# CyberAgentAILab/layout-dm

Hardware: NVIDIA H100
Metric: layouts_per_sec_T100_batch1024_N25 (higher is better)
Workload: dtype fp16

## Files before the change

### layoutdm_b200/csrc/common.cuh

```cuda
#pragma once
#include <cuda.h>
#include <cuda_bf16.h>
#include <cuda_fp16.h>
#include <cuda_runtime.h>
#include <stdint.h>

namespace ldm {

#define LDM_DEVINL __device__ __forceinline__

constexpr float kLogEps = -69.07755278982137f;

LDM_DEVINL uint32_t smem_u32(const void* p) { return static_cast<uint32_t>(__cvta_generic_to_shared(p)); }
LDM_DEVINL void st_shared_u32(uint32_t addr, uint32_t v) { asm volatile("st.shared.u32 [%0], %1;" ::"r"(addr), "r"(v) : "memory"); }

LDM_DEVINL void pdl_wait() { asm volatile("griddepcontrol.wait;" ::: "memory"); }
LDM_DEVINL void pdl_launch_dependents() { asm volatile("griddepcontrol.launch_dependents;" ::: "memory"); }
LDM_DEVINL void pdl_sync() { pdl_wait(); pdl_launch_dependents(); }

LDM_DEVINL void mbar_init(uint64_t* bar, uint32_t count) {
  asm volatile("mbarrier.init.shared::cta.b64 [%0], %1;" ::"r"(smem_u32(bar)), "r"(count) : "memory");
}
LDM_DEVINL void fence_mbar_init() { asm volatile("fence.mbarrier_init.release.cluster;" ::: "memory"); }

// ... 35 lines not shown
               ::"l"(reinterpret_cast<uint64_t>(map)), "r"(smem_u32(smem_src)), "r"(c0), "r"(c1)
               : "memory");
}
LDM_DEVINL void bulk_copy_g2s(void* smem_dst, const void* src, uint32_t bytes, uint64_t* bar) {
  asm volatile("cp.async.bulk.shared::cluster.global.mbarrier::complete_tx::bytes [%0], [%1], %2, [%3];"
               ::"r"(smem_u32(smem_dst)), "l"(reinterpret_cast<uint64_t>(src)), "r"(bytes), "r"(smem_u32(bar))
               : "memory");
}
LDM_DEVINL void bulk_copy_s2g(void* dst, const void* smem_src, uint32_t bytes) {
  asm volatile("cp.async.bulk.global.shared::cta.bulk_group [%0], [%1], %2;"
               ::"l"(reinterpret_cast<uint64_t>(dst)), "r"(smem_u32(smem_src)), "r"(bytes)
               : "memory");
}
LDM_DEVINL void bulk_commit_group() { asm volatile("cp.async.bulk.commit_group;" ::: "memory"); }
template <int N>
LDM_DEVINL void bulk_wait_group_read() { asm volatile("cp.async.bulk.wait_group.read %0;" ::"n"(N) : "memory"); }
LDM_DEVINL void bulk_wait_group_all() { asm volatile("cp.async.bulk.wait_group 0;" ::: "memory"); }
LDM_DEVINL void fence_proxy_async_smem() { asm volatile("fence.proxy.async.shared::cta;" ::: "memory"); }

template <int R>
LDM_DEVINL void setmaxnreg_inc() { asm volatile("setmaxnreg.inc.sync.aligned.u32 %0;" ::"n"(R)); }
template <int R>
LDM_DEVINL void setmaxnreg_dec() { asm volatile("setmaxnreg.dec.sync.aligned.u32 %0;" ::"n"(R)); }

LDM_DEVINL void named_bar_sync(int id, int nthreads) { asm volatile("bar.sync %0, %1;" ::"r"(id), "r"(nthreads) : "memory"); }
LDM_DEVINL void named_bar_arrive(int id, int nthreads) { asm volatile("bar.arrive %0, %1;" ::"r"(id), "r"(nthreads) : "memory"); }

LDM_DEVINL void wgmma_fence() { asm volatile("wgmma.fence.sync.aligned;" ::: "memory"); }
LDM_DEVINL void wgmma_commit() { asm volatile("wgmma.commit_group.sync.aligned;" ::: "memory"); }
template <int N>
LDM_DEVINL void wgmma_wait() { asm volatile("wgmma.wait_group.sync.aligned %0;" ::"n"(N) : "memory"); }
template <int N>
LDM_DEVINL void fence_acc(float (&d)[N]) {
#pragma unroll
  for (int i = 0; i < N; ++i) asm volatile("" : "+f"(d[i])::"memory");
}

template <int SW>
LDM_DEVINL uint64_t make_smem_desc(uint32_t smem_addr) {
  static_assert(SW == 128 || SW == 64, "the kernels use the 128- and 64-byte swizzles");
  uint64_t d = 0;
  d |= static_cast<uint64_t>((smem_addr & 0x3FFFF) >> 4);
  d |= static_cast<uint64_t>(1) << 16;
  d |= static_cast<uint64_t>(8 * SW >> 4) << 32;
  d |= static_cast<uint64_t>(SW == 128 ? 1 : 2) << 62;
  return d;
// ... 215 lines not shown
```

### layoutdm_b200/csrc/gemm_tc.cuh

```cuda
#pragma once
#include "common.cuh"

namespace ldm {

constexpr int kBM = 128;
constexpr int kWgK = 16;
constexpr int kGemmConsumers = 256;
constexpr int kProducerRegs = 40, kConsumerRegs = 232;

constexpr int gemm_kb(bool split) { return split ? 32 : 64; }

enum : int { EPI_QKV = 0, EPI_RELU = 1, EPI_F32 = 2, EPI_LN = 3 };

struct GemmParams {
  int M, N, K;
  int n_tiles;
  const float* bias;
  void* out;
  int ldo;
  float qscale;
  int qcols;
  const float* resid;
  float* y_out;
  const float* ln_scale;
// ... 437 lines not shown
          for (int h = 0; h < 2; ++h) {
            float v[4];
            bias_act<EPI>(acc[h], j8, p.bias, c, scale, v);
            st_shared_u32(blk + (h * 64 + rw) * 128, O::pack(v[0], v[1]));
            st_shared_u32(blk + (h * 64 + rw + 8) * 128, O::pack(v[2], v[3]));
          }
        }
        fence_proxy_async_smem();
        wg_bar();
        if (leader) {
          tma_store_2d(&map_out, stage, n0 + cb * 64, m0);
          bulk_commit_group();
        }
      }
    }
    if (!mine_any) {
      for (int kb = 0; kb < num_kb; ++kb) { mbar_wait(&a_full[kb], ip); mbar_arrive(&a_empty[kb]); }
    }
  }
  if (leader) bulk_wait_group_all();
}

constexpr int kLnThreads = 384, kLnEpiThreads = 96;
struct LnSmem {
  static constexpr int kRows = 64, kWgCols = 232, kCols = 2 * kWgCols;
  using R = Ring<32, 1, kRows, kWgCols, 2, 3, false>;
  static constexpr int kLd = kCols + 8;
  static constexpr int kOffBuf = R::kBytes;
  static constexpr int kOffBars = kOffBuf + kRows * kLd * 4;
  static constexpr int kOffStat = kOffBars + 64;
  static constexpr int kBytes = kOffStat + 3 * kRows * 4 + 1024 ;
  static_assert(kLd * 4 % 16 == 0, "bulk copies need 16-byte aligned rows");
  static_assert(kBytes <= 232448, "exceeds the 227 KB of shared memory per CTA");
};

template <int MODE>
__global__ void __launch_bounds__(kLnThreads, 1)
gemm_ln_kernel(const __grid_constant__ OpMaps<MODE> map_a , const __grid_constant__ OpMaps<MODE> map_b ,
               const GemmParams p) {
  static_assert(!kOpSplit<MODE>, "the split mode runs the fragment-epilogue LN GEMM");
  using SM = LnSmem;
  using O = OpT<MODE>;
  constexpr int kRows = SM::kRows, kWgCols = SM::kWgCols, kLd = SM::kLd, kAcc = kWgCols / 2;
  constexpr int kEpi = kGemmConsumers, kProducer = kEpi + kLnEpiThreads;

  extern __shared__ __align__(1024) uint8_t smem_raw[];
  uint8_t* smem = reinterpret_cast<uint8_t*>((reinterpret_cast<uintptr_t>(smem_raw) + 1023) & ~uintptr_t(1023));
  SM::R ring(smem, reinterpret_cast<uint64_t*>(smem + SM::kOffBars));
  uint64_t* res_full = ring.empty + SM::R::kStages;
  uint64_t* buf_full = res_full + 1;
  float* buf = reinterpret_cast<float*>(smem + SM::kOffBuf);
  float* s_piv = reinterpret_cast<float*>(smem + SM::kOffStat);
  float* s_sum = s_piv + kRows;
  float* s_rstd = s_sum + kRows;

  const int warp = __shfl_sync(0xffffffffu, threadIdx.x >> 5, 0), lane = threadIdx.x & 31;
  const int N = p.N;
  const int num_kb = SM::R::num_kb(p.K);
  const int n_work = p.M / kRows;
  const auto tile_m0 = [&](int t) { return (p.rev ? n_work - 1 - t : t) * kRows; };

  if (threadIdx.x == kProducer) {
    ring.prefetch(map_a, map_b);
    ring.init();
    mbar_init(res_full, 1);
    mbar_init(buf_full, kGemmConsumers);
    fence_mbar_init();
  }
  __syncthreads();
  pdl_sync();

  if (threadIdx.x >= kProducer) {
    if (threadIdx.x == kProducer) {
      uint32_t phase = 0;
      int s = 0;
      for (int t = blockIdx.x; t < n_work; t += gridDim.x) ring.load_tile(s, phase, map_a, map_b, num_kb, tile_m0(t), 0);
    }
    return;
  }

  if (threadIdx.x >= kEpi) {
    const int et = threadIdx.x - kEpi;
    const bool copier = et < 32;
    const uint32_t row_bytes = static_cast<uint32_t>(N) * sizeof(float);
    const float inv_n = 1.0f / static_cast<float>(N);
    constexpr int kVec = kWgCols / 2;
    constexpr int kTotal = kRows * kVec;
    constexpr int kPerThread = (kTotal + kLnEpiThreads - 1) / kLnEpiThreads;
    const auto load_resid = [&](int t) {
      if (lane == 0) mbar_arrive_expect_tx(res_full, kRows * row_bytes);
      __syncwarp();
      const float* src = p.resid + static_cast<size_t>(tile_m0(t)) * N;
      for (int r = lane; r < kRows; r += 32) bulk_copy_g2s(buf + r * kLd, src + static_cast<size_t>(r) * N, row_bytes, res_full);
    };
    const auto store_rows = [&](float* dst) {
      for (int r = lane; r < kRows; r += 32) bulk_copy_s2g(dst + static_cast<size_t>(r) * N, buf + r * kLd, row_bytes);
      bulk_commit_group();
    };
    if (copier) load_resid(blockIdx.x);
    uint32_t bphase = 0;
    for (int t = blockIdx.x; t < n_work; t += gridDim.x) {
      const int m0 = tile_m0(t);
      mbar_wait(buf_full, bphase);
      if (copier && p.y_out != nullptr) store_rows(p.y_out + static_cast<size_t>(m0) * N);
      {
        const int h = (lane >> 2) & 1, q = lane & 3;
#pragma unroll 1
        for (int g = et >> 5; g < kRows / 4; g += kLnEpiThreads / 32) {
          const int r = 4 * g + (lane >> 3);
          const float piv = s_piv[r];
          const float* yr = buf + r * kLd + h * kWgCols + 2 * q;
          float s = 0.0f;
#pragma unroll
          for (int j = 0; j < kWgCols / 8; ++j) {
            const float2 y = *reinterpret_cast<const float2*>(yr + 8 * j);
            s += (y.x - piv) + (y.y - piv);
          }
          s += __shfl_xor_sync(0xffffffffu, s, 1);
          s += __shfl_xor_sync(0xffffffffu, s, 2);
          s += __shfl_xor_sync(0xffffffffu, s, 4);
          float v = 0.0f;
#pragma unroll
          for (int j = 0; j < kWgCols / 8; ++j) {
            const float2 y = *reinterpret_cast<const float2*>(yr + 8 * j);
            const float d0 = fmaf(-s, inv_n, y.x - piv), d1 = fmaf(-s, inv_n, y.y - piv);
            v = fmaf(d0, d0, fmaf(d1, d1, v));
          }
          v += __shfl_xor_sync(0xffffffffu, v, 1);
          v += __shfl_xor_sync(0xffffffffu, v, 2);
          v += __shfl_xor_sync(0xffffffffu, v, 4);
          if ((lane & 7) == 0) { s_sum[r] = s; s_rstd[r] = 1.0f / sqrtf(fmaxf(v * inv_n, 0.0f) + 1e-5f); }
        }
      }
      if (copier) bulk_wait_group_read<0>();
      named_bar_sync(1, kLnEpiThreads);
      const LnAffine a = ln_affine(p.ln_scale, p.ln_shift, p.adaln, p.t_layout, p.n_layouts, m0, N);
      typename O::T* out16 = static_cast<typename O::T*>(p.out);
      const bool keep32 = p.out32 != nullptr;
#pragma unroll 6
      for (int k = 0; k < kPerThread; ++k) {
        const int i = k * kLnEpiThreads + et, r = i / kVec, c = (i - r * kVec) * 4;
        if (i >= kTotal) continue;
        float4* bp = reinterpret_cast<float4*>(buf + r * kLd + c);
        const float4 y = *bp;
        const float4 g = __ldg(reinterpret_cast<const float4*>(a.gam + c)), b = __ldg(reinterpret_cast<const float4*>(a.bet + c));
        const float piv = s_piv[r], s = s_sum[r], rstd = s_rstd[r];
        const float4 v = make_float4(fmaf(fmaf(-s, inv_n, y.x - piv) * rstd, g.x + a.gadd, b.x), fmaf(fmaf(-s, inv_n, y.y - piv) * rstd, g.y + a.gadd, b.y),
                                     fmaf(fmaf(-s, inv_n, y.z - piv) * rstd, g.z + a.gadd, b.z), fmaf(fmaf(-s, inv_n, y.w - piv) * rstd, g.w + a.gadd, b.w));
        *reinterpret_cast<uint2*>(out16 + static_cast<size_t>(m0 + r) * N + c) = make_uint2(O::pack(v.x, v.y), O::pack(v.z, v.w));
        if (keep32) *bp = v;
      }
      if (keep32) fence_proxy_async_smem();
      named_bar_sync(1, kLnEpiThreads);
      if (copier) {
        if (keep32) store_rows(p.out32 + static_cast<size_t>(m0) * N);
        bulk_wait_group_read<0>();
        if (t + static_cast<int>(gridDim.x) < n_work) load_resid(t + gridDim.x);
      }
      bphase ^= 1;
    }
    if (copier) bulk_wait_group_all();
    return;
  }

  const int wn = warp >> 2;
  float acc[kAcc];
  int s = 0;
  uint32_t phase = 0, bphase = 0;
  const int rw = (warp & 3) * 16 + (lane >> 2);
  const int cw = wn * kWgCols + 2 * (lane & 3);
  float* bw = buf + rw * kLd + cw;
  for (int t = blockIdx.x; t < n_work; t += gridDim.x) {
    ring.mma_tile<MODE>(s, phase, acc, 0, wn, num_kb, p.K);
    mbar_wait(res_full, bphase);
    if (cw == 0) { const float b0 = __ldg(p.bias); s_piv[rw] = b0 + bw[0]; s_piv[rw + 8] = b0 + bw[8 * kLd]; }
#pragma unroll
    for (int j = 0; j < kAcc / 4; ++j) {
      const float2 b = __ldg(reinterpret_cast<const float2*>(p.bias + cw + 8 * j));
      float2* y0 = reinterpret_cast<float2*>(bw + 8 * j);
      float2* y1 = reinterpret_cast<float2*>(bw + 8 * kLd + 8 * j);
      const float2 r0 = *y0, r1 = *y1;
      *y0 = make_float2(acc[4 * j] + (b.x + r0.x), acc[4 * j + 1] + (b.y + r0.y));
      *y1 = make_float2(acc[4 * j + 2] + (b.x + r1.x), acc[4 * j + 3] + (b.y + r1.y));
    }
    fence_proxy_async_smem();
    mbar_arrive(buf_full);
    bphase ^= 1;
  }
}

}
```

### layoutdm_b200/csrc/ldm_b200.cu

```cuda
#include <cuda.h>
#include <cuda_runtime.h>

#include <algorithm>
#include <cmath>
#include <cstdarg>
#include <cstdio>
#include <cstdlib>
#include <cstring>
#include <type_traits>
#include <vector>

#include "../../include/ldm_b200.h"
#include "attention.cuh"
#include "common.cuh"
#include "embed.cuh"
#include "gemm_tc.cuh"
#include "posterior_sample.cuh"
#include "relation.cuh"

using namespace ldm;

namespace {

thread_local char g_err[512] = "";
int fail(int code, const char* fmt, ...) {
  va_list ap; va_start(ap, fmt); vsnprintf(g_err, sizeof(g_err), fmt, ap); va_end(ap);
  return code;
}
#define CK(call)                                                                                   \
  do {                                                                                             \
    cudaError_t e__ = (call);                                                                      \
    if (e__ != cudaSuccess) return fail(LDM_ERR_CUDA, "%s failed: %s (%s:%d)", #call, cudaGetErrorString(e__), __FILE__, __LINE__); \
  } while (0)

constexpr int kMaxLayers = 16;
constexpr int kHeadPad = 64;
constexpr int kQkvN = 3 * 8 * kHeadPad;
constexpr int kAttN = 8 * kHeadPad;
constexpr int kMaxLayouts = 32767;
constexpr int kLogitLd = 160;
constexpr int kDModel = 464;
constexpr int kPlainBN = 256, kPlainStages = 4;
constexpr int kRbCols = RbSmem::kCols;
static_assert(kDModel <= RbSmem::kAKb * RbSmem::kKB && kAttN % kRbCols == 0 && kQkvN % 64 == 0 && 4 * kDModel % 64 == 0,
              "row-block GEMM shapes: K fits the resident A, Q tiles are whole tiles, N is whole 64-column store blocks");
constexpr int kHeadBN = 160, kHeadStages = 4;
constexpr int kLnBN = 232, kLnStages = 3;
constexpr int kLnKB = LnSmem::R::kKB;
static_assert(LnSmem::kWgCols == kLnBN && kAttN % kLnKB == 0 && 4 * kDModel % kLnKB == 0 && gemm_kb(true) == kLnKB, "LN GEMM shapes");
template <int EPI, int MODE> constexpr auto kGemmPlainSplit = gemm_tc_kernel<kPlainBN, 2, kPlainStages, EPI, MODE>;
template <int MODE> constexpr auto kGemmHead = gemm_tc_kernel<kHeadBN, 2, kHeadStages, EPI_F32, MODE>;
template <int MODE> constexpr auto kGemmLn = gemm_tc_kernel<kLnBN, 1, kLnStages, EPI_LN, MODE>;
constexpr int kPlainSmem = GemmSmem<kPlainBN, 2, kPlainStages, true>::kBytes;
constexpr int kHeadSmem = GemmSmem<kHeadBN, 2, kHeadStages>::kBytes;
constexpr int kLnSmem = GemmSmem<kLnBN, 1, kLnStages>::kBytes;
static_assert(GemmSmem<kHeadBN, 2, kHeadStages, true>::kBytes == kHeadSmem && GemmSmem<kLnBN, 1, kLnStages, true>::kBytes == kLnSmem,
              "split-mode ring stages must keep the one-plane sizes");

using EncodeTiledFn = CUresult (*)(CUtensorMap*, CUtensorMapDataType, cuuint32_t, void*, const cuuint64_t*, const cuuint64_t*,
                                   const cuuint32_t*, const cuuint32_t*, CUtensorMapInterleave, CUtensorMapSwizzle,
                                   CUtensorMapL2promotion, CUtensorMapFloatOOBfill);
EncodeTiledFn g_encode = nullptr;

int load_encode() {
  if (g_encode) return LDM_OK;
  void* fn = nullptr;
  cudaDriverEntryPointQueryResult qres;
  CK(cudaGetDriverEntryPoint("cuTensorMapEncodeTiled", &fn, cudaEnableDefault, &qres));
  if (qres != cudaDriverEntryPointSuccess || fn == nullptr) return fail(LDM_ERR_CUDA, "cuTensorMapEncodeTiled not available");
  g_encode = reinterpret_cast<EncodeTiledFn>(fn);
  return LDM_OK;
}
// ... 49 lines not shown
  float *hlnw = nullptr, *hlnb = nullptr;
  CUtensorMap m_wqkv[kMaxLayers], m_wo[kMaxLayers], m_w1[kMaxLayers], m_w2[kMaxLayers], m_whead;
  void *wqkv_lo[kMaxLayers] = {}, *wo_lo[kMaxLayers] = {}, *w1_lo[kMaxLayers] = {}, *w2_lo[kMaxLayers] = {}, *whead_lo = nullptr;
  CUtensorMap m_wqkv_lo[kMaxLayers], m_wo_lo[kMaxLayers], m_w1_lo[kMaxLayers], m_w2_lo[kMaxLayers], m_whead_lo;
  int *qmap = nullptr, *amap = nullptr, *hmap = nullptr;
  int cap = 0;
  void *x16 = nullptr, *qkv16 = nullptr, *att16 = nullptr, *z16 = nullptr, *hid16 = nullptr;
  float *x32 = nullptr, *y32 = nullptr, *logits = nullptr;
  float* rel_lp = nullptr;
  long long* ids[2] = {nullptr, nullptr};
  long long* ids_final = nullptr;
  long long *c_seq = nullptr, *c_seq_orig = nullptr; unsigned char* c_mask = nullptr; float* c_tbl = nullptr;
  CUtensorMap m_x16, m_z16, m_qkv16;
  CUtensorMap m_att16, m_hid16;
  CUtensorMap m_qkv16_st, m_hid16_st;
  void *x16_lo = nullptr, *qkv16_lo = nullptr, *att16_lo = nullptr, *z16_lo = nullptr, *hid16_lo = nullptr;
  CUtensorMap m_x16_lo, m_z16_lo, m_qkv16_lo, m_att16_lo, m_hid16_lo;
  std::vector<void*> owned;
  int use_graph = 1;
  int sweep = 1;
  int num_sms = 0;
  int max_threads_sm = 0;
  int gemm_ctas = 0;
  int gemm_split = 0;
  int fuse_embed = 1;
  cudaStream_t cap_stream = nullptr;
  cudaGraphExec_t graph_exec = nullptr;
  uint64_t graph_key = 0;
  unsigned long long* call_block = nullptr;
  uint64_t ws_generation = 0;
  int64_t graph_launches = 0;
  std::vector<void*> staging;
};

namespace {

template <typename T>
int dev_alloc(LdmHandle* h, T** p, size_t n) {
  CK(cudaMalloc(reinterpret_cast<void**>(p), n * sizeof(T)));
  h->owned.push_back(*p);
  return LDM_OK;
}
template <typename T>
int dev_upload(LdmHandle* h, T** p, const T* src, size_t n) {
  int rc = dev_alloc(h, p, n);
  if (rc) return rc;
// ... 114 lines not shown
    out[3 * TT + i] = static_cast<float>(std::log(a));
    out[4 * TT + i] = static_cast<float>(std::log(b));
    out[5 * TT + i] = static_cast<float>(std::log(c));
    out[7 * TT + i] = static_cast<float>(l1m(std::log(c)));
  }
}

enum : int { CAT_EMBED = 0, CAT_QKV, CAT_ATTN, CAT_OUTPROJ, CAT_FF1, CAT_FF2, CAT_HEAD, CAT_EPILOGUE, CAT_MISC, CAT_COUNT };

struct ProfScope {
  LdmHandle* h; cudaStream_t st; cudaEvent_t b = nullptr;
  ProfScope(LdmHandle* h_, int cat, cudaStream_t st_) : h(h_), st(st_) {
    h->launches++;
    if (h->prof) {
      cudaEvent_t a; cudaEventCreate(&a); cudaEventCreate(&b);
      cudaEventRecord(a, st);
      h->prof_recs.push_back({cat, a, b});
    }
  }
  ~ProfScope() { if (b) cudaEventRecord(b, st); }
};

template <typename... KArgs, typename... Args>
cudaError_t launch_step(const LdmHandle* h, void (*kernel)(KArgs...), dim3 grid, int block, int smem, cudaStream_t st, Args&&... args) {
  cudaLaunchConfig_t cfg = {};
  cfg.gridDim = grid; cfg.blockDim = dim3(block); cfg.dynamicSmemBytes = smem; cfg.stream = st;
  cudaLaunchAttribute at[1];
  cfg.attrs = at; cfg.numAttrs = 0;
  if (h->pdl) { at[0].id = cudaLaunchAttributeProgrammaticStreamSerialization; at[0].val.programmaticStreamSerializationAllowed = 1; cfg.numAttrs = 1; }
  return cudaLaunchKernelEx(&cfg, kernel, std::forward<Args>(args)...);
}

template <int MODE>
int set_smem() {
  constexpr auto attr = cudaFuncAttributeMaxDynamicSharedMemorySize;
  if constexpr (kOpSplit<MODE>) {
    CK(cudaFuncSetAttribute(kGemmPlainSplit<EPI_QKV, MODE>, attr, kPlainSmem));
    CK(cudaFuncSetAttribute(kGemmPlainSplit<EPI_RELU, MODE>, attr, kPlainSmem));
  } else {
    CK(cudaFuncSetAttribute(gemm_rowblock_kernel<EPI_QKV, MODE>, attr, RbSmem::kBytes));
    CK(cudaFuncSetAttribute(gemm_rowblock_kernel<EPI_RELU, MODE>, attr, RbSmem::kBytes));
  }
  CK(cudaFuncSetAttribute(kGemmHead<MODE>, attr, kHeadSmem));
  if constexpr (kOpSplit<MODE>) CK(cudaFuncSetAttribute(kGemmLn<MODE>, attr, kLnSmem));
  else CK(cudaFuncSetAttribute(gemm_ln_kernel<MODE>, attr, LnSmem::kBytes));
  CK(cudaFuncSetAttribute(attention_kernel<MODE>, attr, kOpSplit<MODE> ? kAttSmemBytesSplit : kAttSmemBytes));
  return LDM_OK;
}

void free_workspace(LdmHandle* h) {
  void** ws[] = {&h->x16, &h->qkv16, &h->att16, &h->z16, &h->hid16, &h->x16_lo, &h->qkv16_lo, &h->att16_lo, &h->z16_lo, &h->hid16_lo,
                 reinterpret_cast<void**>(&h->x32), reinterpret_cast<void**>(&h->y32),
                 reinterpret_cast<void**>(&h->logits), reinterpret_cast<void**>(&h->ids[0]), reinterpret_cast<void**>(&h->ids[1]),
                 reinterpret_cast<void**>(&h->ids_final), reinterpret_cast<void**>(&h->c_seq), reinterpret_cast<void**>(&h->c_seq_orig),
                 reinterpret_cast<void**>(&h->c_mask), reinterpret_cast<void**>(&h->rel_lp)};
  for (void** p : ws) { if (*p) cudaFree(*p); *p = nullptr; }
  h->cap = 0;
}

int ensure_workspace(LdmHandle* h, int n_layouts) {
  if (n_layouts > kMaxLayouts) return fail(LDM_ERR_UNSUPPORTED, "batch of %d layouts exceeds the %d a call supports", n_layouts, kMaxLayouts);
  if (n_layouts <= h->cap) return LDM_OK;
  CK(cudaDeviceSynchronize());
  free_workspace(h);
  const size_t M = static_cast<size_t>(n_layouts) * kBM;
  const int d = h->desc.d_model, ff = h->desc.d_ff;
  if (h->split) {
    void** lo[] = {&h->x16_lo, &h->qkv16_lo, &h->att16_lo, &h->z16_lo, &h->hid16_lo};
    const size_t cols[] = {static_cast<size_t>(d), static_cast<size_t>(kQkvN), static_cast<size_t>(kAttN), static_cast<size_t>(d), static_cast<size_t>(ff)};
// ... 13 lines not shown
  CK(cudaMalloc(&h->z16, M * d * 2));
  CK(cudaMalloc(&h->hid16, M * ff * 2));
  CK(cudaMalloc(reinterpret_cast<void**>(&h->x32), M * d * 4));
  CK(cudaMalloc(reinterpret_cast<void**>(&h->y32), M * d * 4));
  CK(cudaMalloc(reinterpret_cast<void**>(&h->logits), M * kLogitLd * 4));
  const size_t nid = static_cast<size_t>(n_layouts) * h->S;
  CK(cudaMalloc(reinterpret_cast<void**>(&h->ids[0]), nid * 8));
  CK(cudaMalloc(reinterpret_cast<void**>(&h->ids[1]), nid * 8));
  CK(cudaMalloc(reinterpret_cast<void**>(&h->ids_final), nid * 8));
  CK(cudaMalloc(reinterpret_cast<void**>(&h->c_seq), nid * 8));
  CK(cudaMalloc(reinterpret_cast<void**>(&h->c_seq_orig), nid * 8));
  CK(cudaMalloc(reinterpret_cast<void**>(&h->c_mask), nid));
  CK(cudaMemset(h->x16, 0, M * d * 2)); CK(cudaMemset(h->qkv16, 0, M * kQkvN * 2)); CK(cudaMemset(h->att16, 0, M * kAttN * 2));
  CK(cudaMemset(h->z16, 0, M * d * 2)); CK(cudaMemset(h->hid16, 0, M * ff * 2)); CK(cudaMemset(h->x32, 0, M * d * 4));
  CK(cudaMemset(h->y32, 0, M * d * 4));
  CK(cudaMemset(h->logits, 0, M * kLogitLd * 4));
  h->cap = n_layouts;
  h->ws_generation++;
  int rc;
  static_assert(gemm_kb(false) == RbSmem::kKB, "one A geometry for QKV / FF1 / head");
  const int kb = gemm_kb(h->split);
  if ((rc = make_op_maps(h, &h->m_x16, &h->m_x16_lo, h->x16, h->x16_lo, M, d, kBM, kb))) return rc;
  if ((rc = make_op_maps(h, &h->m_z16, &h->m_z16_lo, h->z16, h->z16_lo, M, d, kBM, kb))) return rc;
  if ((rc = make_op_maps(h, &h->m_att16, &h->m_att16_lo, h->att16, h->att16_lo, M, kAttN, 64, kLnKB))) return rc;
  if ((rc = make_op_maps(h, &h->m_hid16, &h->m_hid16_lo, h->hid16, h->hid16_lo, M, ff, 64, kLnKB))) return rc;
  if ((rc = make_op_maps(h, &h->m_qkv16, &h->m_qkv16_lo, h->qkv16, h->qkv16_lo, M, kQkvN, kBM, kHeadPad))) return rc;
  if (!h->split && (rc = make_map(&h->m_qkv16_st, h->qkv16, M, kQkvN, kBM, 64, h->bf16))) return rc;
  if (!h->split && (rc = make_map(&h->m_hid16_st, h->hid16, M, ff, kBM, 64, h->bf16))) return rc;
  return LDM_OK;
}

template <int MODE>
int launch_denoiser(LdmHandle* h, int n, const long long* ids_in, int t_model, cudaStream_t st, const int* t_layout = nullptr, bool skip_embed = false) {
  const auto maps = [](const CUtensorMap& hi, const CUtensorMap& lo) { return op_maps<MODE>(hi, lo); };
  const int d = h->desc.d_model, ff = h->desc.d_ff, L = h->L, T = h->T;
  const int M = n * kBM;
  const auto grid = [&](int tiles, bool persistent) {
    if (!persistent) return dim3(tiles);
    return dim3(std::min({tiles, h->num_sms, h->gemm_ctas > 0 ? h->gemm_ctas : tiles}));
  };
  const auto plain_gemm = [&](auto epi, const OpMaps<MODE>& a, const OpMaps<MODE>& w, const CUtensorMap& out, GemmParams p) {
    constexpr int EPI = decltype(epi)::value;
    if constexpr (kOpSplit<MODE>) {
      p.n_tiles = (p.N + kPlainBN - 1) / kPlainBN;
      return launch_step(h, kGemmPlainSplit<EPI, MODE>, grid(p.n_tiles * n, false), kGemmThreads, kPlainSmem, st, a, w, p);
    } else {
      p.n_tiles = (p.N + kRbCols - 1) / kRbCols;
      const int g = h->gemm_split > 0 ? h->gemm_split : n >= h->num_sms ? 1 : (h->num_sms + n - 1) / n;
      p.n_ranges = std::min(g, p.n_tiles);
      return launch_step(h, gemm_rowblock_kernel<EPI, MODE>, grid(n * p.n_ranges, true), kRbThreads, RbSmem::kBytes, st, a, w, out, p);
    }
  };
  const auto ln_gemm = [&](const OpMaps<MODE>& a, const OpMaps<MODE>& w, const GemmParams& p) {
    if constexpr (kOpSplit<MODE>) return launch_step(h, kGemmLn<MODE>, grid(M / 64, false), kGemmThreads, kLnSmem, st, a, w, p);
    else return launch_step(h, gemm_ln_kernel<MODE>, grid(M / 64, true), kLnThreads, LnSmem::kBytes, st, a, w, p);
  };
  int done = 0;
  int dir = 0;
  auto next_rev = [&]() { dir ^= 1; return h->sweep ? dir : 0; };
#define LDM_STAGE_DONE() do { if (h->debug_stop_after && ++done >= h->debug_stop_after) { CK(cudaGetLastError()); return LDM_OK; } } while (0)
  if (!skip_embed) {
    const int warps = n * 128, blocks = (warps * 32 + 255) / 256;
    ProfScope ps(h, CAT_EMBED, st);
    CK(launch_step(h, embed_adaln_kernel<MODE>, dim3(blocks), 256, 0, st, ids_in, (const float*)h->cat_emb, (const float*)h->pos,
                   (const float*)h->adaln, t_model, t_layout, h->x32, h->x16, n, n, h->S, d, h->x16_lo));
  }
  if (!skip_embed) LDM_STAGE_DONE();
  for (int l = 0; l < L; ++l) {
    {
      GemmParams p{M, kQkvN, d, 0, h->bqkv[l], h->qkv16, kQkvN, 1.0f / sqrtf(static_cast<float>(d / h->desc.n_heads)), 8 * kHeadPad};
      p.rev = next_rev(); p.out_lo = h->qkv16_lo;
      ProfScope ps(h, CAT_QKV, st);
      CK(plain_gemm(std::integral_constant<int, EPI_QKV>{}, maps(h->m_x16, h->m_x16_lo), maps(h->m_wqkv[l], h->m_wqkv_lo[l]), h->m_qkv16_st, p));
    }
    LDM_STAGE_DONE();
    {
      ProfScope ps(h, CAT_ATTN, st);
      CK(launch_step(h, attention_kernel<MODE>, dim3(n * h->desc.n_heads), kAttThreads, kOpSplit<MODE> ? kAttSmemBytesSplit : kAttSmemBytes, st,
// ... 265 lines not shown

  LdmWeights staged{};
  for (const WeightField& f : weight_fields(h)) {
    float* p = nullptr;
    TRY(dev_upload_tmp(h, &p, w->*f.member, f.n));
    staged.*f.member = p;
  }
  TRY(pack_weights(h, staged, nullptr));
  {
    std::vector<float> sch(static_cast<size_t>(h->G) * 8 * (T + 1));
    for (int g = 0; g < h->G; ++g) {
      const int N = desc->q_type == 0 ? (g == 0 ? desc->n_cat : desc->n_bins) + 1 : C - 1;
      build_schedule(*desc, N, sch.data() + static_cast<size_t>(g) * 8 * (T + 1));
    }
    TRY(dev_upload(h, &h->sched, sch.data(), sch.size()));
    TRY(dev_alloc(h, &h->lae, static_cast<size_t>(h->G) * (T + 1) * 4));
    TRY(dev_alloc(h, &h->call_block, static_cast<size_t>(6)));
    lae_table_kernel<<<(h->G * (T + 1) + 127) / 128, 128>>>(h->sched, h->lae, h->G, T + 1);
    if (cudaGetLastError() != cudaSuccess) { ldm_destroy(h); return fail(LDM_ERR_CUDA, "lae_table_kernel launch failed"); }
  }
  if (cudaDeviceSynchronize() != cudaSuccess) { ldm_destroy(h); return fail(LDM_ERR_CUDA, "weight packing failed: %s", cudaGetErrorString(cudaGetLastError())); }
  free_staging(h);

  TRY(h->mode == OP_BF16X3 ? set_smem<OP_BF16X3>() : h->mode == OP_BF16 ? set_smem<OP_BF16>() : set_smem<OP_F16>());
#undef TRY
  *out = h;
  return LDM_OK;
}

int ldm_destroy(LdmHandle* h) {
  if (!h) return LDM_OK;
  cudaSetDevice(h->desc.device);
  cudaDeviceSynchronize();
  if (h->graph_exec) cudaGraphExecDestroy(h->graph_exec);
  if (h->cap_stream) cudaStreamDestroy(h->cap_stream);
  for (void* p : h->owned) cudaFree(p);
  free_staging(h);
  free_workspace(h);
  if (h->c_tbl) cudaFree(h->c_tbl);
  delete h;
  return LDM_OK;
}

int ldm_load_weights(LdmHandle* h, const LdmWeights* w, void* stream) {
  if (!h || !w) return fail(LDM_ERR_INVALID, "null argument");
  CK(cudaSetDevice(h->desc.device));
  for (const WeightField& f : weight_fields(h)) {
// ... 439 lines not shown
```

Measured before the change: 1048.

## Split LN GEMM columns across a 2-CTA cluster with DSMEM stat exchange

Restructures the fused GEMM+LayerNorm kernel so that each CTA pair in a cluster computes 128 rows by half the model width (232 columns). Partial row sums and variances are exchanged through distributed shared memory using st.async and mbarriers. Both consumer warpgroups now split rows instead of columns, and the row sum moves into the consumer epilogue. Stage counts differ per GEMM (out-proj vs FF2), and the persistent grid is sized from cluster occupancy. This aims to double M per tile and lower per-CTA smem for the weight ring, at the cost of cluster synchronisation and cross-CTA latency.

```diff
diff --git a/layoutdm_b200/csrc/common.cuh b/layoutdm_b200/csrc/common.cuh
--- a/layoutdm_b200/csrc/common.cuh
+++ b/layoutdm_b200/csrc/common.cuh
@@ -81,6 +81,21 @@
 LDM_DEVINL void setmaxnreg_inc() { asm volatile("setmaxnreg.inc.sync.aligned.u32 %0;" ::"n"(R)); }
 template <int R>
 LDM_DEVINL void setmaxnreg_dec() { asm volatile("setmaxnreg.dec.sync.aligned.u32 %0;" ::"n"(R)); }
+
+LDM_DEVINL uint32_t cluster_ctarank() { uint32_t r; asm volatile("mov.u32 %0, %%cluster_ctarank;" : "=r"(r)); return r; }
+LDM_DEVINL uint32_t cluster_id_x() { uint32_t r; asm volatile("mov.u32 %0, %%clusterid.x;" : "=r"(r)); return r; }
+LDM_DEVINL uint32_t cluster_count_x() { uint32_t r; asm volatile("mov.u32 %0, %%nclusterid.x;" : "=r"(r)); return r; }
+LDM_DEVINL void cluster_sync() {
+  asm volatile("barrier.cluster.arrive.release;\n\tbarrier.cluster.wait.acquire;" ::: "memory");
+}
+LDM_DEVINL uint32_t map_peer(const void* p, uint32_t rank) {
+  uint32_t r;
+  asm volatile("mapa.shared::cluster.u32 %0, %1, %2;" : "=r"(r) : "r"(smem_u32(p)), "r"(rank));
+  return r;
+}
+LDM_DEVINL void st_async_f32(uint32_t addr, float v, uint32_t bar) {
+  asm volatile("st.async.shared::cluster.mbarrier::complete_tx::bytes.f32 [%0], %1, [%2];" ::"r"(addr), "f"(v), "r"(bar) : "memory");
+}
 
 LDM_DEVINL void named_bar_sync(int id, int nthreads) { asm volatile("bar.sync %0, %1;" ::"r"(id), "r"(nthreads) : "memory"); }
 LDM_DEVINL void named_bar_arrive(int id, int nthreads) { asm volatile("bar.arrive %0, %1;" ::"r"(id), "r"(nthreads) : "memory"); }
diff --git a/layoutdm_b200/csrc/gemm_tc.cuh b/layoutdm_b200/csrc/gemm_tc.cuh
--- a/layoutdm_b200/csrc/gemm_tc.cuh
+++ b/layoutdm_b200/csrc/gemm_tc.cuh
@@ -483,120 +483,133 @@
 }
 
 constexpr int kLnThreads = 384, kLnEpiThreads = 96;
+template <int STAGES>
 struct LnSmem {
-  static constexpr int kRows = 64, kWgCols = 232, kCols = 2 * kWgCols;
-  using R = Ring<32, 1, kRows, kWgCols, 2, 3, false>;
-  static constexpr int kLd = kCols + 8;
+  static constexpr int kRows = kBM, kCols = 232, kPairCols = 2 * kCols;
+  using R = Ring<32, 1, kRows, kCols, 1, STAGES, false>;
+  static constexpr int kLd = kCols;
   static constexpr int kOffBuf = R::kBytes;
   static constexpr int kOffBars = kOffBuf + kRows * kLd * 4;
-  static constexpr int kOffStat = kOffBars + 64;
-  static constexpr int kBytes = kOffStat + 3 * kRows * 4 + 1024 ;
-  static_assert(kLd * 4 % 16 == 0, "bulk copies need 16-byte aligned rows");
-  static_assert(kBytes <= 232448, "exceeds the 227 KB of shared memory per CTA");
+  static constexpr int kOffStat = kOffBars + 128;
+  static constexpr int kBytes = kOffStat + 9 * kRows * 4 + 1024 ;
+  static_assert(2 * R::kStages * 8 + 6 * 8 <= 128, "barrier block overflow");
+  static_assert(kLd * 4 % 16 == 0 && kLd * 4 % 128 == 32, "bulk copies need 16-byte aligned rows; fragment accesses need rows 32 mod 128 bytes");
+  static_assert(kRows * kCols * 4 < (1 << 20), "a tile's residual bytes exceed the mbarrier transaction count");
 };
 
-template <int MODE>
+template <int MODE, int STAGES>
 __global__ void __launch_bounds__(kLnThreads, 1)
 gemm_ln_kernel(const __grid_constant__ OpMaps<MODE> map_a , const __grid_constant__ OpMaps<MODE> map_b ,
                const GemmParams p) {
   static_assert(!kOpSplit<MODE>, "the split mode runs the fragment-epilogue LN GEMM");
-  using SM = LnSmem;
+  using SM = LnSmem<STAGES>;
   using O = OpT<MODE>;
-  constexpr int kRows = SM::kRows, kWgCols = SM::kWgCols, kLd = SM::kLd, kAcc = kWgCols / 2;
+  constexpr int kRows = SM::kRows, kCols = SM::kCols, kLd = SM::kLd, kAcc = kCols / 2;
   constexpr int kEpi = kGemmConsumers, kProducer = kEpi + kLnEpiThreads;
 
   extern __shared__ __align__(1024) uint8_t smem_raw[];
   uint8_t* smem = reinterpret_cast<uint8_t*>((reinterpret_cast<uintptr_t>(smem_raw) + 1023) & ~uintptr_t(1023));
-  SM::R ring(smem, reinterpret_cast<uint64_t*>(smem + SM::kOffBars));
+  typename SM::R ring(smem, reinterpret_cast<uint64_t*>(smem + SM::kOffBars));
   uint64_t* res_full = ring.empty + SM::R::kStages;
   uint64_t* buf_full = res_full + 1;
+  uint64_t* xs_full = buf_full + 1;
+  uint64_t* xv_full = xs_full + 2;
   float* buf = reinterpret_cast<float*>(smem + SM::kOffBuf);
   float* s_piv = reinterpret_cast<float*>(smem + SM::kOffStat);
-  float* s_sum = s_piv + kRows;
-  float* s_rstd = s_sum + kRows;
+  float* s_own = s_piv + kRows;
+  float* s_sum = s_own + kRows;
+  float* v_own = s_sum + kRows;
+  float* s_rstd = v_own + kRows;
+  float* x_sum = s_rstd + kRows;
+  float* x_var = x_sum + 2 * kRows;
 
   const int warp = __shfl_sync(0xffffffffu, threadIdx.x >> 5, 0), lane = threadIdx.x & 31;
   const int N = p.N;
   const int num_kb = SM::R::num_kb(p.K);
   const int n_work = p.M / kRows;
+  const uint32_t rank = cluster_ctarank();
+  const int col0 = kCols * static_cast<int>(rank);
+  const int cl = static_cast<int>(cluster_id_x()), n_cl = static_cast<int>(cluster_count_x());
   const auto tile_m0 = [&](int t) { return (p.rev ? n_work - 1 - t : t) * kRows; };
+  const uint32_t peer = rank ^ 1;
+  const uint32_t px_sum = map_peer(x_sum, peer), pxs_full = map_peer(xs_full, peer);
 
   if (threadIdx.x == kProducer) {
     ring.prefetch(map_a, map_b);
     ring.init();
     mbar_init(res_full, 1);
     mbar_init(buf_full, kGemmConsumers);
+    for (int b = 0; b < 2; ++b) { mbar_init(&xs_full[b], 1); mbar_init(&xv_full[b], 1); }
     fence_mbar_init();
   }
-  __syncthreads();
+  cluster_sync();
   pdl_sync();
 
   if (threadIdx.x >= kProducer) {
     if (threadIdx.x == kProducer) {
       uint32_t phase = 0;
       int s = 0;
-      for (int t = blockIdx.x; t < n_work; t += gridDim.x) ring.load_tile(s, phase, map_a, map_b, num_kb, tile_m0(t), 0);
-    }
-    return;
-  }
-
-  if (threadIdx.x >= kEpi) {
+      for (int t = cl; t < n_work; t += n_cl) ring.load_tile(s, phase, map_a, map_b, num_kb, tile_m0(t), col0);
+    }
+  } else if (threadIdx.x >= kEpi) {
     const int et = threadIdx.x - kEpi;
     const bool copier = et < 32;
-    const uint32_t row_bytes = static_cast<uint32_t>(N) * sizeof(float);
+    constexpr uint32_t kRowBytes = kCols * sizeof(float);
     const float inv_n = 1.0f / static_cast<float>(N);
-    constexpr int kVec = kWgCols / 2;
+    constexpr int kVec = kCols / 4;
     constexpr int kTotal = kRows * kVec;
     constexpr int kPerThread = (kTotal + kLnEpiThreads - 1) / kLnEpiThreads;
+    const uint32_t px_var = map_peer(x_var, peer), pxv_full = map_peer(xv_full, peer);
     const auto load_resid = [&](int t) {
-      if (lane == 0) mbar_arrive_expect_tx(res_full, kRows * row_bytes);
+      if (lane == 0) mbar_arrive_expect_tx(res_full, kRows * kRowBytes);
       __syncwarp();
-      const float* src = p.resid + static_cast<size_t>(tile_m0(t)) * N;
-      for (int r = lane; r < kRows; r += 32) bulk_copy_g2s(buf + r * kLd, src + static_cast<size_t>(r) * N, row_bytes, res_full);
+      const float* src = p.resid + static_cast<size_t>(tile_m0(t)) * N + col0;
+      for (int r = lane; r < kRows; r += 32) bulk_copy_g2s(buf + r * kLd, src + static_cast<size_t>(r) * N, kRowBytes, res_full);
     };
     const auto store_rows = [&](float* dst) {
-      for (int r = lane; r < kRows; r += 32) bulk_copy_s2g(dst + static_cast<size_t>(r) * N, buf + r * kLd, row_bytes);
+      for (int r = lane; r < kRows; r += 32) bulk_copy_s2g(dst + static_cast<size_t>(r) * N, buf + r * kLd, kRowBytes);
       bulk_commit_group();
     };
-    if (copier) load_resid(blockIdx.x);
+    if (copier) load_resid(cl);
     uint32_t bphase = 0;
-    for (int t = blockIdx.x; t < n_work; t += gridDim.x) {
-      const int m0 = tile_m0(t);
+    int it = 0;
+    for (int t = cl; t < n_work; t += n_cl, ++it) {
+      const int m0 = tile_m0(t), b = it & 1;
+      const uint32_t xph = (it >> 1) & 1;
+      if (et == 0) { mbar_arrive_expect_tx(&xs_full[b], kRows * 4); mbar_arrive_expect_tx(&xv_full[b], kRows * 4); }
       mbar_wait(buf_full, bphase);
-      if (copier && p.y_out != nullptr) store_rows(p.y_out + static_cast<size_t>(m0) * N);
-      {
-        const int h = (lane >> 2) & 1, q = lane & 3;
+      if (copier && p.y_out != nullptr) store_rows(p.y_out + static_cast<size_t>(m0) * N + col0);
+      const int q = lane & 3;
+      mbar_wait(&xs_full[b], xph);
 #pragma unroll 1
-        for (int g = et >> 5; g < kRows / 4; g += kLnEpiThreads / 32) {
-          const int r = 4 * g + (lane >> 3);
-          const float piv = s_piv[r];
-          const float* yr = buf + r * kLd + h * kWgCols + 2 * q;
-          float s = 0.0f;
-#pragma unroll
-          for (int j = 0; j < kWgCols / 8; ++j) {
-            const float2 y = *reinterpret_cast<const float2*>(yr + 8 * j);
-            s += (y.x - piv) + (y.y - piv);
-          }
-          s += __shfl_xor_sync(0xffffffffu, s, 1);
-          s += __shfl_xor_sync(0xffffffffu, s, 2);
-          s += __shfl_xor_sync(0xffffffffu, s, 4);
-          float v = 0.0f;
-#pragma unroll
-          for (int j = 0; j < kWgCols / 8; ++j) {
-            const float2 y = *reinterpret_cast<const float2*>(yr + 8 * j);
-            const float d0 = fmaf(-s, inv_n, y.x - piv), d1 = fmaf(-s, inv_n, y.y - piv);
-            v = fmaf(d0, d0, fmaf(d1, d1, v));
-          }
-          v += __shfl_xor_sync(0xffffffffu, v, 1);
-          v += __shfl_xor_sync(0xffffffffu, v, 2);
-          v += __shfl_xor_sync(0xffffffffu, v, 4);
-          if ((lane & 7) == 0) { s_sum[r] = s; s_rstd[r] = 1.0f / sqrtf(fmaxf(v * inv_n, 0.0f) + 1e-5f); }
+      for (int g = et >> 5; g < kRows / 8; g += kLnEpiThreads / 32) {
+        const int r = 8 * g + (lane >> 2);
+        const float piv = s_piv[r], s = s_own[r] + x_sum[b * kRows + r];
+        const float* yr = buf + r * kLd + 2 * q;
+        float v = 0.0f;
+#pragma unroll
+        for (int j = 0; j < kCols / 8; ++j) {
+          const float2 y = *reinterpret_cast<const float2*>(yr + 8 * j);
+          const float d0 = fmaf(-s, inv_n, y.x - piv), d1 = fmaf(-s, inv_n, y.y - piv);
+          v = fmaf(d0, d0, fmaf(d1, d1, v));
+        }
+        v += __shfl_xor_sync(0xffffffffu, v, 1);
+        v += __shfl_xor_sync(0xffffffffu, v, 2);
+        if (q == 0) { s_sum[r] = s; v_own[r] = v; st_async_f32(px_var + (b * kRows + r) * 4, v, pxv_full + b * 8); }
+      }
+      mbar_wait(&xv_full[b], xph);
+      if (q == 0) {
+#pragma unroll 1
+        for (int g = et >> 5; g < kRows / 8; g += kLnEpiThreads / 32) {
+          const int r = 8 * g + (lane >> 2);
+          s_rstd[r] = 1.0f / sqrtf(fmaxf((v_own[r] + x_var[b * kRows + r]) * inv_n, 0.0f) + 1e-5f);
         }
       }
       if (copier) bulk_wait_group_read<0>();
       named_bar_sync(1, kLnEpiThreads);
       const LnAffine a = ln_affine(p.ln_scale, p.ln_shift, p.adaln, p.t_layout, p.n_layouts, m0, N);
-      typename O::T* out16 = static_cast<typename O::T*>(p.out);
+      const float *gam = a.gam + col0, *bet = a.bet + col0;
+      typename O::T* out16 = static_cast<typename O::T*>(p.out) + col0;
       const bool keep32 = p.out32 != nullptr;
 #pragma unroll 6
       for (int k = 0; k < kPerThread; ++k) {
@@ -604,50 +617,76 @@
         if (i >= kTotal) continue;
         float4* bp = reinterpret_cast<float4*>(buf + r * kLd + c);
         const float4 y = *bp;
-        const float4 g = __ldg(reinterpret_cast<const float4*>(a.gam + c)), b = __ldg(reinterpret_cast<const float4*>(a.bet + c));
+        const float4 g = __ldg(reinterpret_cast<const float4*>(gam + c)), h = __ldg(reinterpret_cast<const float4*>(bet + c));
         const float piv = s_piv[r], s = s_sum[r], rstd = s_rstd[r];
-        const float4 v = make_float4(fmaf(fmaf(-s, inv_n, y.x - piv) * rstd, g.x + a.gadd, b.x), fmaf(fmaf(-s, inv_n, y.y - piv) * rstd, g.y + a.gadd, b.y),
-                                     fmaf(fmaf(-s, inv_n, y.z - piv) * rstd, g.z + a.gadd, b.z), fmaf(fmaf(-s, inv_n, y.w - piv) * rstd, g.w + a.gadd, b.w));
+        const float4 v = make_float4(fmaf(fmaf(-s, inv_n, y.x - piv) * rstd, g.x + a.gadd, h.x), fmaf(fmaf(-s, inv_n, y.y - piv) * rstd, g.y + a.gadd, h.y),
+                                     fmaf(fmaf(-s, inv_n, y.z - piv) * rstd, g.z + a.gadd, h.z), fmaf(fmaf(-s, inv_n, y.w - piv) * rstd, g.w + a.gadd, h.w));
         *reinterpret_cast<uint2*>(out16 + static_cast<size_t>(m0 + r) * N + c) = make_uint2(O::pack(v.x, v.y), O::pack(v.z, v.w));
         if (keep32) *bp = v;
       }
       if (keep32) fence_proxy_async_smem();
       named_bar_sync(1, kLnEpiThreads);
       if (copier) {
-        if (keep32) store_rows(p.out32 + static_cast<size_t>(m0) * N);
+        if (keep32) store_rows(p.out32 + static_cast<size_t>(m0) * N + col0);
         bulk_wait_group_read<0>();
-        if (t + static_cast<int>(gridDim.x) < n_work) load_resid(t + gridDim.x);
+        if (t + n_cl < n_work) load_resid(t + n_cl);
       }
       bphase ^= 1;
     }
     if (copier) bulk_wait_group_all();
-    return;
-  }
-
-  const int wn = warp >> 2;
-  float acc[kAcc];
-  int s = 0;
-  uint32_t phase = 0, bphase = 0;
-  const int rw = (warp & 3) * 16 + (lane >> 2);
-  const int cw = wn * kWgCols + 2 * (lane & 3);
-  float* bw = buf + rw * kLd + cw;
-  for (int t = blockIdx.x; t < n_work; t += gridDim.x) {
-    ring.mma_tile<MODE>(s, phase, acc, 0, wn, num_kb, p.K);
-    mbar_wait(res_full, bphase);
-    if (cw == 0) { const float b0 = __ldg(p.bias); s_piv[rw] = b0 + bw[0]; s_piv[rw + 8] = b0 + bw[8 * kLd]; }
-#pragma unroll
-    for (int j = 0; j < kAcc / 4; ++j) {
-      const float2 b = __ldg(reinterpret_cast<const float2*>(p.bias + cw + 8 * j));
-      float2* y0 = reinterpret_cast<float2*>(bw + 8 * j);
-      float2* y1 = reinterpret_cast<float2*>(bw + 8 * kLd + 8 * j);
-      const float2 r0 = *y0, r1 = *y1;
-      *y0 = make_float2(acc[4 * j] + (b.x + r0.x), acc[4 * j + 1] + (b.y + r0.y));
-      *y1 = make_float2(acc[4 * j + 2] + (b.x + r1.x), acc[4 * j + 3] + (b.y + r1.y));
-    }
-    fence_proxy_async_smem();
-    mbar_arrive(buf_full);
-    bphase ^= 1;
-  }
+  } else {
+    const int wg = warp >> 2;
+    float acc[kAcc];
+    int s = 0;
+    uint32_t phase = 0, bphase = 0;
+    const int rw = 64 * wg + (warp & 3) * 16 + (lane >> 2);
+    const int cw = 2 * (lane & 3);
+    const float* bias = p.bias + col0;
+    float* bw = buf + rw * kLd + cw;
+    int it = 0;
+    for (int t = cl; t < n_work; t += n_cl, ++it) {
+      const int m0 = tile_m0(t);
+      ring.template mma_tile<MODE>(s, phase, acc, wg, 0, num_kb, p.K);
+      float piv0 = 0.0f, piv1 = 0.0f;
+      if (cw == 0) {
+        const float b0 = __ldg(p.bias);
+        piv0 = b0 + p.resid[static_cast<size_t>(m0 + rw) * N];
+        piv1 = b0 + p.resid[static_cast<size_t>(m0 + rw + 8) * N];
+      }
+      piv0 = __shfl_sync(0xffffffffu, piv0, lane & ~3);
+      piv1 = __shfl_sync(0xffffffffu, piv1, lane & ~3);
+      mbar_wait(res_full, bphase);
+      if (cw == 0) { s_piv[rw] = piv0; s_piv[rw + 8] = piv1; }
+      float s0 = 0.0f, s1 = 0.0f;
+#pragma unroll
+      for (int j = 0; j < kAcc / 4; ++j) {
+        const float2 b = __ldg(reinterpret_cast<const float2*>(bias + cw + 8 * j));
+        float2* y0 = reinterpret_cast<float2*>(bw + 8 * j);
+        float2* y1 = reinterpret_cast<float2*>(bw + 8 * kLd + 8 * j);
+        const float2 r0 = *y0, r1 = *y1;
+        const float2 v0 = make_float2(acc[4 * j] + (b.x + r0.x), acc[4 * j + 1] + (b.y + r0.y));
+        const float2 v1 = make_float2(acc[4 * j + 2] + (b.x + r1.x), acc[4 * j + 3] + (b.y + r1.y));
+        *y0 = v0;
+        *y1 = v1;
+        s0 += (v0.x - piv0) + (v0.y - piv0);
+        s1 += (v1.x - piv1) + (v1.y - piv1);
+      }
+      s0 += __shfl_xor_sync(0xffffffffu, s0, 1);
+      s1 += __shfl_xor_sync(0xffffffffu, s1, 1);
+      s0 += __shfl_xor_sync(0xffffffffu, s0, 2);
+      s1 += __shfl_xor_sync(0xffffffffu, s1, 2);
+      if (cw == 0) {
+        const int b = it & 1;
+        s_own[rw] = s0; s_own[rw + 8] = s1;
+        st_async_f32(px_sum + (b * kRows + rw) * 4, s0, pxs_full + b * 8);
+        st_async_f32(px_sum + (b * kRows + rw + 8) * 4, s1, pxs_full + b * 8);
+      }
+      fence_proxy_async_smem();
+      mbar_arrive(buf_full);
+      bphase ^= 1;
+    }
+  }
+  cluster_sync();
 }
 
 }
diff --git a/layoutdm_b200/csrc/ldm_b200.cu b/layoutdm_b200/csrc/ldm_b200.cu
--- a/layoutdm_b200/csrc/ldm_b200.cu
+++ b/layoutdm_b200/csrc/ldm_b200.cu
@@ -46,8 +46,13 @@
               "row-block GEMM shapes: K fits the resident A, Q tiles are whole tiles, N is whole 64-column store blocks");
 constexpr int kHeadBN = 160, kHeadStages = 4;
 constexpr int kLnBN = 232, kLnStages = 3;
-constexpr int kLnKB = LnSmem::R::kKB;
-static_assert(LnSmem::kWgCols == kLnBN && kAttN % kLnKB == 0 && 4 * kDModel % kLnKB == 0 && gemm_kb(true) == kLnKB, "LN GEMM shapes");
+constexpr int kLnSplitRows = 64;
+constexpr int kLnOutStages = 3, kLnFf2Stages = 4;
+using LnOut = LnSmem<kLnOutStages>;
+using LnFf2 = LnSmem<kLnFf2Stages>;
+constexpr int kLnKB = LnFf2::R::kKB;
+static_assert(LnOut::R::kKB == kLnKB && LnFf2::kCols == kLnBN && LnFf2::kPairCols == kDModel && kAttN % kLnKB == 0 &&
+              4 * kDModel % kLnKB == 0 && gemm_kb(true) == kLnKB, "LN GEMM shapes");
 template <int EPI, int MODE> constexpr auto kGemmPlainSplit = gemm_tc_kernel<kPlainBN, 2, kPlainStages, EPI, MODE>;
 template <int MODE> constexpr auto kGemmHead = gemm_tc_kernel<kHeadBN, 2, kHeadStages, EPI_F32, MODE>;
 template <int MODE> constexpr auto kGemmLn = gemm_tc_kernel<kLnBN, 1, kLnStages, EPI_LN, MODE>;
@@ -143,6 +148,7 @@
   int num_sms = 0;
   int max_threads_sm = 0;
   int gemm_ctas = 0;
+  int ln_clusters = 0;
   int gemm_split = 0;
   int fuse_embed = 1;
   cudaStream_t cap_stream = nullptr;
@@ -303,17 +309,22 @@
 };
 
 template <typename... KArgs, typename... Args>
-cudaError_t launch_step(const LdmHandle* h, void (*kernel)(KArgs...), dim3 grid, int block, int smem, cudaStream_t st, Args&&... args) {
+cudaError_t launch_cluster(const LdmHandle* h, int cluster, void (*kernel)(KArgs...), dim3 grid, int block, int smem, cudaStream_t st, Args&&... args) {
   cudaLaunchConfig_t cfg = {};
   cfg.gridDim = grid; cfg.blockDim = dim3(block); cfg.dynamicSmemBytes = smem; cfg.stream = st;
-  cudaLaunchAttribute at[1];
+  cudaLaunchAttribute at[2];
   cfg.attrs = at; cfg.numAttrs = 0;
-  if (h->pdl) { at[0].id = cudaLaunchAttributeProgrammaticStreamSerialization; at[0].val.programmaticStreamSerializationAllowed = 1; cfg.numAttrs = 1; }
+  if (h->pdl) { at[cfg.numAttrs].id = cudaLaunchAttributeProgrammaticStreamSerialization; at[cfg.numAttrs++].val.programmaticStreamSerializationAllowed = 1; }
+  if (cluster > 1) { at[cfg.numAttrs].id = cudaLaunchAttributeClusterDimension; at[cfg.numAttrs++].val.clusterDim = {static_cast<unsigned>(cluster), 1, 1}; }
   return cudaLaunchKernelEx(&cfg, kernel, std::forward<Args>(args)...);
 }
+template <typename... KArgs, typename... Args>
+cudaError_t launch_step(const LdmHandle* h, void (*kernel)(KArgs...), dim3 grid, int block, int smem, cudaStream_t st, Args&&... args) {
+  return launch_cluster(h, 1, kernel, grid, block, smem, st, std::forward<Args>(args)...);
+}
 
 template <int MODE>
-int set_smem() {
+int set_smem(LdmHandle* h) {
   constexpr auto attr = cudaFuncAttributeMaxDynamicSharedMemorySize;
   if constexpr (kOpSplit<MODE>) {
     CK(cudaFuncSetAttribute(kGemmPlainSplit<EPI_QKV, MODE>, attr, kPlainSmem));
@@ -324,8 +335,20 @@
   }
   CK(cudaFuncSetAttribute(kGemmHead<MODE>, attr, kHeadSmem));
   if constexpr (kOpSplit<MODE>) CK(cudaFuncSetAttribute(kGemmLn<MODE>, attr, kLnSmem));
-  else CK(cudaFuncSetAttribute(gemm_ln_kernel<MODE>, attr, LnSmem::kBytes));
+  else {
+    CK(cudaFuncSetAttribute(gemm_ln_kernel<MODE, kLnOutStages>, attr, LnOut::kBytes));
+    CK(cudaFuncSetAttribute(gemm_ln_kernel<MODE, kLnFf2Stages>, attr, LnFf2::kBytes));
+  }
   CK(cudaFuncSetAttribute(attention_kernel<MODE>, attr, kOpSplit<MODE> ? kAttSmemBytesSplit : kAttSmemBytes));
+  if constexpr (!kOpSplit<MODE>) {
+    cudaLaunchConfig_t cfg = {};
+    cfg.gridDim = dim3(2); cfg.blockDim = dim3(kLnThreads); cfg.dynamicSmemBytes = LnFf2::kBytes;
+    cudaLaunchAttribute at[1];
+    at[0].id = cudaLaunchAttributeClusterDimension; at[0].val.clusterDim = {2, 1, 1};
+    cfg.attrs = at; cfg.numAttrs = 1;
+    CK(cudaOccupancyMaxActiveClusters(&h->ln_clusters, gemm_ln_kernel<MODE, kLnFf2Stages>, &cfg));
+    if (h->ln_clusters < 1) return fail(LDM_ERR_UNSUPPORTED, "gemm_ln_kernel: no CTA pair of %d bytes of shared memory fits the device", LnFf2::kBytes);
+  }
   return LDM_OK;
 }
 
@@ -385,8 +408,9 @@
   const int kb = gemm_kb(h->split);
   if ((rc = make_op_maps(h, &h->m_x16, &h->m_x16_lo, h->x16, h->x16_lo, M, d, kBM, kb))) return rc;
   if ((rc = make_op_maps(h, &h->m_z16, &h->m_z16_lo, h->z16, h->z16_lo, M, d, kBM, kb))) return rc;
-  if ((rc = make_op_maps(h, &h->m_att16, &h->m_att16_lo, h->att16, h->att16_lo, M, kAttN, 64, kLnKB))) return rc;
-  if ((rc = make_op_maps(h, &h->m_hid16, &h->m_hid16_lo, h->hid16, h->hid16_lo, M, ff, 64, kLnKB))) return rc;
+  const int ln_rows = h->split ? kLnSplitRows : LnFf2::kRows;
+  if ((rc = make_op_maps(h, &h->m_att16, &h->m_att16_lo, h->att16, h->att16_lo, M, kAttN, ln_rows, kLnKB))) return rc;
+  if ((rc = make_op_maps(h, &h->m_hid16, &h->m_hid16_lo, h->hid16, h->hid16_lo, M, ff, ln_rows, kLnKB))) return rc;
   if ((rc = make_op_maps(h, &h->m_qkv16, &h->m_qkv16_lo, h->qkv16, h->qkv16_lo, M, kQkvN, kBM, kHeadPad))) return rc;
   if (!h->split && (rc = make_map(&h->m_qkv16_st, h->qkv16, M, kQkvN, kBM, 64, h->bf16))) return rc;
   if (!h->split && (rc = make_map(&h->m_hid16_st, h->hid16, M, ff, kBM, 64, h->bf16))) return rc;
@@ -415,8 +439,13 @@
     }
   };
   const auto ln_gemm = [&](const OpMaps<MODE>& a, const OpMaps<MODE>& w, const GemmParams& p) {
-    if constexpr (kOpSplit<MODE>) return launch_step(h, kGemmLn<MODE>, grid(M / 64, false), kGemmThreads, kLnSmem, st, a, w, p);
-    else return launch_step(h, gemm_ln_kernel<MODE>, grid(M / 64, true), kLnThreads, LnSmem::kBytes, st, a, w, p);
+    if constexpr (kOpSplit<MODE>) {
+      return launch_step(h, kGemmLn<MODE>, grid(M / kLnSplitRows, false), kGemmThreads, kLnSmem, st, a, w, p);
+    } else {
+      const int pairs = std::min({n, h->ln_clusters, h->gemm_ctas > 0 ? std::max(1, h->gemm_ctas / 2) : n});
+      if (p.K == kAttN) return launch_cluster(h, 2, gemm_ln_kernel<MODE, kLnOutStages>, dim3(2 * pairs), kLnThreads, LnOut::kBytes, st, a, w, p);
+      return launch_cluster(h, 2, gemm_ln_kernel<MODE, kLnFf2Stages>, dim3(2 * pairs), kLnThreads, LnFf2::kBytes, st, a, w, p);
+    }
   };
   int done = 0;
   int dir = 0;
@@ -728,7 +757,7 @@
   if (cudaDeviceSynchronize() != cudaSuccess) { ldm_destroy(h); return fail(LDM_ERR_CUDA, "weight packing failed: %s", cudaGetErrorString(cudaGetLastError())); }
   free_staging(h);
 
-  TRY(h->mode == OP_BF16X3 ? set_smem<OP_BF16X3>() : h->mode == OP_BF16 ? set_smem<OP_BF16>() : set_smem<OP_F16>());
+  TRY(h->mode == OP_BF16X3 ? set_smem<OP_BF16X3>(h) : h->mode == OP_BF16 ? set_smem<OP_BF16>(h) : set_smem<OP_F16>(h));
 #undef TRY
   *out = h;
   return LDM_OK;
```

New measurement: 1088 (median of 6 runs). +3.8%, better.
